# harmony-one/harmony

Hardware: AMD Instinct MI355X
Metric: BLS12-381 aggregate-verifies/sec (committee=4096) (higher is better)
Workload: dtype u64; 1 GPU; config2: committee=4096 masked aggregate + pairing verify, batch=262144/step, masks Bernoulli(0.9) seed 42, 48B staking commit payloads; parallelism=dp1 (per-shard replicas, no collective)

## Files before the change

### harmony_amd/core.py

```python
import ctypes
import os

_DIR = os.path.dirname(os.path.abspath(__file__))
_SO = os.environ.get("HBLS_SO", os.path.join(_DIR, "libhbls.so"))

HBLS_OK = 1
HBLS_FALSE = 0
HBLS_ERR = -1
HBLS_ERR_NOGPU = -2
HBLS_ERR_BADINPUT = -3
HBLS_NOQUORUM = -4
NOQUORUM = HBLS_NOQUORUM
TWO_THIRDS_DEC = 666666666666666667


class HblsError(RuntimeError):
    pass


class NoGpuError(HblsError):
    pass


class BadInputError(HblsError, ValueError):
# ... 35 lines not shown
                                       ctypes.c_size_t, ctypes.c_char_p]
    lib.hbls_msm_g1_committee.argtypes = [ctypes.c_void_p, ctypes.c_char_p,
                                          ctypes.c_char_p]
    lib.hbls_batch_agg_verify_partials.argtypes = [
        ctypes.c_void_p, ctypes.c_char_p, ctypes.c_char_p, ctypes.c_size_t,
        ctypes.c_char_p, ctypes.c_char_p, ctypes.c_size_t, ctypes.c_size_t,
        ctypes.POINTER(ctypes.c_int32)]
    lib.hbls_stream_create.restype = ctypes.c_void_p
    lib.hbls_stream_create.argtypes = [ctypes.c_void_p, ctypes.c_int]
    lib.hbls_stream_free.argtypes = [ctypes.c_void_p]
    lib.hbls_stream_set_rounds.argtypes = [
        ctypes.c_void_p, ctypes.POINTER(ctypes.c_uint32), ctypes.c_int,
        ctypes.c_char_p, ctypes.c_size_t]
    lib.hbls_stream_process.argtypes = [
        ctypes.c_void_p, ctypes.POINTER(ctypes.c_uint32),
        ctypes.POINTER(ctypes.c_uint32), ctypes.c_char_p,
        ctypes.POINTER(ctypes.c_uint32), ctypes.c_int,
        ctypes.c_size_t, ctypes.POINTER(ctypes.c_int32)]
    lib.hbls_stream_check.argtypes = [
        ctypes.c_void_p, ctypes.POINTER(ctypes.c_uint32), ctypes.c_int,
        ctypes.POINTER(ctypes.c_int32)]
    lib.hbls_stream_check_submit.argtypes = [
        ctypes.c_void_p, ctypes.POINTER(ctypes.c_uint32), ctypes.c_int]
    lib.hbls_stream_check_poll.argtypes = [
        ctypes.c_void_p, ctypes.POINTER(ctypes.c_int32)]
    lib.hbls_stream_get.argtypes = [ctypes.c_void_p, ctypes.c_uint32,
                                    ctypes.c_char_p, ctypes.c_char_p]
    lib.hbls_stream_set_verify_mode.argtypes = [ctypes.c_void_p, ctypes.c_int]
    lib.hbls_batch_verify_votes_grouped.argtypes = [
        ctypes.c_void_p, ctypes.POINTER(ctypes.c_uint32),
        ctypes.POINTER(ctypes.c_uint32), ctypes.c_char_p, ctypes.c_char_p,
        ctypes.c_size_t, ctypes.c_size_t, ctypes.c_size_t,
        ctypes.POINTER(ctypes.c_int32)]
    lib.hbls_vote_key_sums.argtypes = [
        ctypes.c_void_p, ctypes.POINTER(ctypes.c_uint32),
        ctypes.POINTER(ctypes.c_uint32), ctypes.c_size_t, ctypes.c_char_p,
        ctypes.POINTER(ctypes.c_int32)]
    lib.hbls_batch_verify_votes_multi.argtypes = [
        ctypes.c_void_p, ctypes.POINTER(ctypes.c_uint32),
        ctypes.POINTER(ctypes.c_uint32), ctypes.c_char_p, ctypes.c_char_p,
        ctypes.c_size_t, ctypes.c_size_t, ctypes.POINTER(ctypes.c_int32)]
    lib.hbls_stream_process_multi.argtypes = [
        ctypes.c_void_p, ctypes.POINTER(ctypes.c_uint32),
        ctypes.POINTER(ctypes.c_uint32), ctypes.POINTER(ctypes.c_uint32),
        ctypes.c_char_p, ctypes.POINTER(ctypes.c_uint32), ctypes.c_int,
        ctypes.c_size_t, ctypes.POINTER(ctypes.c_int32)]
    lib.hbls_rlc_last_stats.argtypes = [ctypes.POINTER(ctypes.c_uint32)]
    lib.hbls_rlc_last_stats.restype = None
    lib.hbls_set_agg_verify_mode.argtypes = [ctypes.c_int]
    lib.hbls_set_aggrlc_threshold.argtypes = [ctypes.c_int]
    lib.hbls_set_aggrlc_threshold.restype = None
    lib.hbls_aggrlc_last_stats.argtypes = [ctypes.POINTER(ctypes.c_uint32)]
    lib.hbls_aggrlc_last_stats.restype = None
    u64p, u32p, i32p = (ctypes.POINTER(t) for t in
                        (ctypes.c_uint64, ctypes.c_uint32, ctypes.c_int32))
    lib.hbls_committee_set_quorum.argtypes = [ctypes.c_void_p, u64p, ctypes.c_uint64]
    lib.hbls_mask_power.argtypes = [ctypes.c_void_p, ctypes.c_char_p, ctypes.c_size_t,
                                    u64p, u32p]
    lib.hbls_agg_verify_quorum.argtypes = lib.hbls_agg_verify.argtypes
    lib.hbls_batch_agg_verify_quorum.argtypes = lib.hbls_batch_agg_verify.argtypes
    lib.hbls_batch_seal_verify_quorum.argtypes = lib.hbls_batch_seal_verify.argtypes
    lib.hbls_stream_power.argtypes = [ctypes.c_void_p, u32p, ctypes.c_int,
                                      u64p, u32p, i32p]
    lib.hbls_last_stage_ns.argtypes = [ctypes.c_int]
    lib.hbls_copy_bench_ns.restype = ctypes.c_uint64
    lib.hbls_copy_bench_ns.argtypes = [ctypes.c_size_t]
    lib.hbls_fpmul_bench_waves.restype = ctypes.c_double
    lib.hbls_fpmul_bench_waves.argtypes = [ctypes.c_int, ctypes.c_int]
    return lib


_lib = _load()


def _check(rc, what):
    if rc == HBLS_ERR_NOGPU:
        raise NoGpuError(f"{what}: no AMD GPU available (product path requires gfx950)")
    if rc == HBLS_ERR_BADINPUT:
        raise BadInputError(f"{what}: bad input")
    if rc < 0:
        raise HblsError(f"{what}: error {rc}")
    return rc


def version() -> str:
    return _lib.hbls_version().decode()


def device_count() -> int:
    return _lib.hbls_device_count()


def init(device=-1):
    _check(_lib.hbls_init(device), "hbls_init")


def last_kernel_ns() -> int:
    return _lib.hbls_last_kernel_ns()


def last_stage_ns(i: int) -> int:
    return _lib.hbls_last_stage_ns(i)


def set_g2_cofactor_mode(fast: bool):
    _lib.hbls_set_g2_cofactor_mode(int(fast))


def set_coop_threshold(n: int):
    _lib.hbls_set_coop_threshold(n)


def rlc_chunk_size() -> int:
    return _lib.hbls_rlc_chunk_size()


def rlc_last_stats():
    out = (ctypes.c_uint32 * 4)()
    _lib.hbls_rlc_last_stats(out)
    return list(out)


def set_agg_verify_mode(mode: int):
    _check(_lib.hbls_set_agg_verify_mode(mode), "set_agg_verify_mode")


def set_aggrlc_threshold(n: int):
    _lib.hbls_set_aggrlc_threshold(n)


def aggrlc_chunk_size() -> int:
    return _lib.hbls_aggrlc_chunk_size()


def aggrlc_last_stats():
    out = (ctypes.c_uint32 * 3)()
    _lib.hbls_aggrlc_last_stats(out)
    return list(out)


def pk_from_sk(sk32: bytes) -> bytes:
    out = ctypes.create_string_buffer(48)
    _check(_lib.hbls_pk_from_sk(sk32, out), "pk_from_sk")
    return out.raw


def batch_pk_from_sk(sks: bytes, batch: int) -> bytes:
    out = ctypes.create_string_buffer(48 * batch)
    _check(_lib.hbls_batch_pk_from_sk(sks, batch, out), "batch_pk_from_sk")
    return out.raw


def sign_hash(sk32: bytes, msg: bytes) -> bytes:
    out = ctypes.create_string_buffer(96)
    _check(_lib.hbls_sign_hash(sk32, msg, len(msg), out), "sign_hash")
    return out.raw


def batch_sign(sks: bytes, msgs: bytes, mlen: int, batch: int) -> bytes:
    out = ctypes.create_string_buffer(96 * batch)
    _check(_lib.hbls_batch_sign(sks, msgs, mlen, batch, out), "batch_sign")
    return out.raw


def hash_to_g2(msg: bytes) -> bytes:
    out = ctypes.create_string_buffer(96)
    _check(_lib.hbls_hash_to_g2(msg, len(msg), out), "hash_to_g2")
    return out.raw


def batch_hash_to_g2(msgs: bytes, mlen: int, batch: int) -> bytes:
    out = ctypes.create_string_buffer(96 * batch)
    _check(_lib.hbls_batch_hash_to_g2(msgs, mlen, batch, out), "batch_hash_to_g2")
    return out.raw


def verify_hash(pk48: bytes, sig96: bytes, msg: bytes) -> bool:
    rc = _lib.hbls_verify_hash(pk48, sig96, msg, len(msg))
    return _check(rc, "verify_hash") == HBLS_OK


def g1_add(a: bytes, b: bytes) -> bytes:
    out = ctypes.create_string_buffer(48)
    _check(_lib.hbls_g1_add(a, b, out), "g1_add")
    return out.raw


def g1_sub(a: bytes, b: bytes) -> bytes:
    out = ctypes.create_string_buffer(48)
    _check(_lib.hbls_g1_sub(a, b, out), "g1_sub")
    return out.raw


# ... 334 lines not shown
```

### harmony_amd/csrc/hbls_aggrlc.inc

```

#define AGGRLC_CHUNK 64
#define AGGRLC_WINDOWS 8

__global__ void k_aggrlc_pow2(g1aff_t *p2) {
    int k = blockIdx.x * blockDim.x + threadIdx.x;
    if (k >= 64) return;
    g1_t base, p;
    fp_load(base.x, BLS_G1_X); fp_load(base.y, BLS_G1_Y); fp_one(base.z);
    g1_neg(p, base);
    for (int j = 0; j < k; j++) g1_dbl(p, p);
    g1aff_t a;
    g1_to_affine(a, p);
    p2[k] = a;
}

__global__ void k_aggrlc_miller(const g1_t *aggpubs, const g2_t *hms, const g2aff_t *sigs,
                                const int32_t *sig_flags, const int32_t *hm_ok,
                                const uint64_t *scalars, const g1aff_t *gtab,
                                fp12_t *F, int32_t *elig, int32_t *results, int batch) {
    int i = blockIdx.x * blockDim.x + threadIdx.x;
    if (i >= batch) return;
    fp12_t f;
    fp12_one(f);
    elig[i] = 0;
// ... 30 lines not shown
      fp_mul(zi, ti, A.z);
      fp_sqr(zi2, zi);
      fp_mul(zi3, zi2, zi);
      fp_mul(ca.x, C.x, zi2);
      fp_mul(ca.y, C.y, zi3); }
    g2aff_t ha;
    g2_t hmc = hms[i];
    g2_to_affine(ha, hmc);
    miller_loop2(f, ha, pa, sigs[i], ca);
    F[i] = f;
    elig[i] = 1;
    results[i] = 1;
}

__global__ void __launch_bounds__(AGGRLC_CHUNK) k_aggrlc_chunk_prod(
        const fp12_t *F, const int32_t *elig, int batch, int nchunks,
        fp12_t *FC, int32_t *ccnt, int32_t *cforce) {
    int c = blockIdx.x;
    if (c >= nchunks) return;
    __shared__ fp12_t red[AGGRLC_CHUNK];
    size_t i = (size_t)c * AGGRLC_CHUNK + threadIdx.x;
    int e = i < (size_t)batch ? elig[i] : 0;
    if (e == 1) red[threadIdx.x] = F[i];
    else fp12_one(red[threadIdx.x]);
    int cnt = __syncthreads_count(e != 0);
    int force = __syncthreads_or(e == 2);
    for (int s = AGGRLC_CHUNK / 2; s > 0; s >>= 1) {
        if (threadIdx.x < s) {
            fp12_t t;
            fp12_mul(t, red[threadIdx.x], red[threadIdx.x + s]);
            red[threadIdx.x] = t;
        }
        __syncthreads();
    }
    if (threadIdx.x == 0) {
        FC[c] = red[0];
        ccnt[c] = cnt;
        cforce[c] = force ? 1 : 0;
    }
}

__global__ void k_aggrlc_final(const fp12_t *FC, const int32_t *ccnt,
                               const int32_t *cforce, int32_t *verdict, int nchunks) {
    int c = blockIdx.x * blockDim.x + threadIdx.x;
    if (c >= nchunks) return;
    if (cforce[c]) { verdict[c] = 0; return; }
    if (ccnt[c] == 0) { verdict[c] = 1; return; }
    fp12_t f = FC[c];
    fp12_conj(f, f);
    final_exp(f, f);
    verdict[c] = fp12_is_one(f) ? 1 : 0;
}

__global__ void k_verify_sel(const uint32_t *sel, int nsel, const g1_t *aggpubs,
                             const g2_t *hms, const g2aff_t *sigs,
                             const int32_t *sig_flags, const int32_t *hm_ok,
                             int32_t *results, int batch) {
    int j = blockIdx.x * blockDim.x + threadIdx.x;
    if (j >= nsel) return;
    uint32_t i = sel[j];
    if (i >= (uint32_t)batch) return;
    if (!hm_ok[i] || sig_flags[i] == 0) { results[i] = HBLS_ERR_BADINPUT; return; }
    g2aff_t dummy;
    bool sig_inf = sig_flags[i] == 2;
    results[i] = verify_pairing(aggpubs[i], hms[i], sig_inf ? dummy : sigs[i], sig_inf);
}


static thread_local uint32_t g_aggrlc_stats[3] = {0, 0, 0};
extern "C" void hbls_aggrlc_last_stats(uint32_t out[3]) {
    for (int i = 0; i < 3; i++) out[i] = g_aggrlc_stats[i];
}
static void aggrlc_stats_reset(void) {
    for (int i = 0; i < 3; i++) g_aggrlc_stats[i] = 0;
}
extern "C" int hbls_aggrlc_chunk_size(void) { return AGGRLC_CHUNK; }

static int g_agg_verify_mode = -2;
#define AGGRLC_DEFAULT_THRESHOLD 131072
static int g_aggrlc_threshold = AGGRLC_DEFAULT_THRESHOLD;
static int agg_verify_mode(void) {
    if (g_agg_verify_mode == -2) {
        const char *e = getenv("HBLS_AGG_VERIFY_MODE");
        int m = e ? atoi(e) : -1;
        g_agg_verify_mode = (m == 0 || m == 1) ? m : -1;
    }
    return g_agg_verify_mode;
}
extern "C" int hbls_set_agg_verify_mode(int mode) {
    if (mode < -1 || mode > 1) return HBLS_ERR_BADINPUT;
    g_agg_verify_mode = mode;
    return HBLS_OK;
}
extern "C" void hbls_set_aggrlc_threshold(int n) {
    g_aggrlc_threshold = n < 0 ? AGGRLC_DEFAULT_THRESHOLD : n;
}

static g1aff_t *g_aggrlc_gtab = nullptr;
static int aggrlc_init_tables(void) {
    if (g_aggrlc_gtab) return HBLS_OK;
    const size_t m = AGGRLC_WINDOWS * 255;
    DevBuf dp2(64 * sizeof(g1aff_t)), dwj(m * sizeof(g1_t)), dwi(m);
    g1aff_t *d_gt = nullptr;
    if (dp2.err || dwj.err || dwi.err) return HBLS_ERR;
    HIP_OK(hipMalloc(&d_gt, m * sizeof(g1aff_t)));
    hipLaunchKernelGGL(k_aggrlc_pow2, dim3(1), dim3(64), 0, 0, dp2.as<g1aff_t>());
    hipLaunchKernelGGL(k_wtab_build_jac, dim3(1), dim3(64), 0, 0,
                       dp2.as<g1aff_t>(), 64, dwj.as<g1_t>(), AGGRLC_WINDOWS);
    hipLaunchKernelGGL(k_wtab_to_affine, dim3((int)((m + 255) / 256)), dim3(256), 0, 0,
                       dwj.as<g1_t>(), d_gt, dwi.as<uint8_t>(), m);
    std::vector<uint8_t> winf(m);
    bool ok = hipDeviceSynchronize() == hipSuccess &&
              hipMemcpy(winf.data(), dwi.p, m, hipMemcpyDeviceToHost) == hipSuccess;
    for (size_t k = 0; ok && k < m; k++)
        if (winf[k]) ok = false;
    if (!ok) { hipFree(d_gt); return HBLS_ERR; }
    g_aggrlc_gtab = d_gt;
    return HBLS_OK;
}

static bool aggrlc_wanted(size_t batch) {
    int m = agg_verify_mode();
    if (m == 0 || !g_aggrlc_gtab) return false;
    if (batch > RLC_MAX_ITEMS || (long long)batch < (long long)g_aggrlc_threshold) return false;
    if (m == 1) return true;
    return (int)batch > coop_threshold() && rf_mode() == 0 && !use_batch_affine();
}

static int aggrlc_verify(const g1_t *d_agg, const g2_t *d_hm, const g2aff_t *d_saff,
                         const int32_t *d_sflags, const int32_t *d_hok,
                         int32_t *d_res, size_t batch) {
    size_t nc = (batch + AGGRLC_CHUNK - 1) / AGGRLC_CHUNK;
    std::vector<uint64_t> scalars(batch);
    if (!rlc_draw_scalars(scalars.data(), batch)) return AGGRLC_FALLBACK;
    DevBuf dsc(batch * 8), dF(batch * sizeof(fp12_t)), delig(batch * 4);
    DevBuf dFC(nc * sizeof(fp12_t)), dcs(3 * nc * 4);
    if (dsc.err || dF.err || delig.err || dFC.err || dcs.err) {
        (void)hipGetLastError();
        return AGGRLC_FALLBACK;
    }
    HIP_OK(hipMemcpy(dsc.p, scalars.data(), batch * 8, hipMemcpyHostToDevice));
    int32_t *d_ccnt = dcs.as<int32_t>(), *d_cforce = d_ccnt + nc, *d_verdict = d_cforce + nc;
    hipEvent_t ev[4];
    for (int i = 0; i < 4; i++) (void)hipEventCreate(&ev[i]);
    (void)hipEventRecord(ev[0], 0);
    hipLaunchKernelGGL(k_aggrlc_miller, dim3((uint32_t)((batch + 63) / 64)), dim3(64), 0, 0,
                       d_agg, d_hm, d_saff, d_sflags, d_hok, dsc.as<uint64_t>(),
                       g_aggrlc_gtab, dF.as<fp12_t>(), delig.as<int32_t>(), d_res, (int)batch);
    (void)hipEventRecord(ev[1], 0);
    hipLaunchKernelGGL(k_aggrlc_chunk_prod, dim3((uint32_t)nc), dim3(AGGRLC_CHUNK), 0, 0,
                       dF.as<fp12_t>(), delig.as<int32_t>(), (int)batch, (int)nc,
                       dFC.as<fp12_t>(), d_ccnt, d_cforce);
    (void)hipEventRecord(ev[2], 0);
    hipLaunchKernelGGL(k_aggrlc_final, dim3((uint32_t)((nc + 63) / 64)), dim3(64), 0, 0,
                       dFC.as<fp12_t>(), d_ccnt, d_cforce, d_verdict, (int)nc);
    (void)hipEventRecord(ev[3], 0);
    std::vector<int32_t> hc(3 * nc);
    hipError_t e = hipMemcpy(hc.data(), dcs.p, 3 * nc * 4, hipMemcpyDeviceToHost);
    if (e == hipSuccess) e = hipGetLastError();
    for (int i = 0; i < 3; i++) {
        float ms = 0;
        if (e == hipSuccess) (void)hipEventElapsedTime(&ms, ev[i], ev[i + 1]);
        g_stage_ns[4 + i] = (uint64_t)(ms * 1e6);
    }
    for (int i = 0; i < 4; i++) (void)hipEventDestroy(ev[i]);
    HIP_OK(e);

    std::vector<uint32_t> failed;
    for (size_t c = 0; c < nc; c++) {
        if (hc[c] <= 0) continue;
        g_aggrlc_stats[0]++;
        if (hc[2 * nc + c] == 1) continue;
        g_aggrlc_stats[1]++;
        failed.push_back((uint32_t)c);
    }
    if (failed.empty()) return HBLS_OK;

    std::vector<int32_t> helig(batch);
    HIP_OK(hipMemcpy(helig.data(), delig.p, batch * 4, hipMemcpyDeviceToHost));
    std::vector<uint32_t> sel;
    for (uint32_t c : failed)
        for (size_t i = (size_t)c * AGGRLC_CHUNK;
             i < batch && i < ((size_t)c + 1) * AGGRLC_CHUNK; i++)
            if (helig[i]) sel.push_back((uint32_t)i);
    size_t ns = sel.size();
    g_aggrlc_stats[2] = (uint32_t)ns;
    if (!ns) return HBLS_OK;
    DevBuf dsel(ns * 4);
    if (dsel.err) return HBLS_ERR;
    HIP_OK(hipMemcpy(dsel.p, sel.data(), ns * 4, hipMemcpyHostToDevice));
    hipLaunchKernelGGL(k_verify_sel, dim3((uint32_t)((ns + 63) / 64)), dim3(64), 0, 0,
                       dsel.as<uint32_t>(), (int)ns, d_agg, d_hm, d_saff, d_sflags, d_hok,
                       d_res, (int)batch);
    HIP_OK(hipGetLastError());
    return HBLS_OK;
}
```

### harmony_amd/csrc/hbls_dev.hip

```cpp
#include <hip/hip_runtime.h>
#include <stdint.h>
#include <string.h>
#include <stdio.h>
#include <stdlib.h>
#include "../../oracle/bls_consts.h"
#include "../../include/hbls.h"

typedef unsigned __int128 u128;

#define DEV __device__ __forceinline__
#define DEVN __device__ __noinline__

struct fp_t { uint64_t l[6]; };
struct fp2_t { fp_t a, b; };

DEV bool fp_is_zero(const fp_t &x) {
    return (x.l[0] | x.l[1] | x.l[2] | x.l[3] | x.l[4] | x.l[5]) == 0;
}
DEV bool fp_eq(const fp_t &x, const fp_t &y) {
    uint64_t d = 0;
#pragma unroll
    for (int i = 0; i < 6; i++) d |= x.l[i] ^ y.l[i];
    return d == 0;
}
// ... 2105 lines not shown
static int aggrlc_init_tables(void);
static bool aggrlc_wanted(size_t batch);
static void aggrlc_stats_reset(void);

#define HIP_OK(expr) do { hipError_t _e = (expr); if (_e != hipSuccess) { \
    fprintf(stderr, "hbls: %s failed: %s\n", #expr, hipGetErrorString(_e)); return HBLS_ERR; } } while (0)
#define HIP_OKP(expr) do { hipError_t _e = (expr); if (_e != hipSuccess) { \
    fprintf(stderr, "hbls: %s failed: %s\n", #expr, hipGetErrorString(_e)); return nullptr; } } while (0)

extern "C" int hbls_device_count(void) {
    int n = 0;
    if (hipGetDeviceCount(&n) != hipSuccess) return 0;
    return n;
}

extern "C" int hbls_init(int device) {
    int n = hbls_device_count();
    if (n <= 0) return HBLS_ERR_NOGPU;
    if (device >= 0) {
        if (device >= n) return HBLS_ERR_BADINPUT;
        if (hipSetDevice(device) != hipSuccess) return HBLS_ERR;
        g_device = device;
    } else {
        hipGetDevice(&g_device);
    }
    void *p = nullptr;
    if (hipMalloc(&p, 64) != hipSuccess) return HBLS_ERR;
    hipFree(p);
    g_init_rc = HBLS_OK;
    (void)aggrlc_init_tables();
    return HBLS_OK;
}

extern "C" void hbls_set_g2_cofactor_mode(int fast) { g_fast_cofactor = fast; }
extern "C" const char *hbls_version(void) { return "hbls 0.1 (gfx950)"; }
extern "C" uint64_t hbls_last_kernel_ns(void) { return g_last_ns; }
extern "C" uint64_t hbls_last_stage_ns(int i) { return (i >= 0 && i < 8) ? g_stage_ns[i] : 0; }

static int require_gpu(void) {
    if (g_init_rc != HBLS_OK) {
        if (hbls_init(-1) != HBLS_OK) return HBLS_ERR_NOGPU;
    }
    return HBLS_OK;
}

struct DevBuf {
    void *p = nullptr;
    hipError_t err = hipSuccess;
    explicit DevBuf(size_t n) { err = hipMalloc(&p, n ? n : 1); }
    ~DevBuf() { if (p) hipFree(p); }
    template <typename T> T *as() const { return (T *)p; }
};

struct Timer {
    hipEvent_t a, b;
    Timer() { hipEventCreate(&a); hipEventCreate(&b); hipEventRecord(a, 0); }
    void stop_and_store() {
        hipEventRecord(b, 0);
        hipEventSynchronize(b);
        float ms = 0;
        hipEventElapsedTime(&ms, a, b);
        g_last_ns = (uint64_t)(ms * 1e6);
        hipEventDestroy(a); hipEventDestroy(b);
    }
};

extern "C" int hbls_batch_pk_from_sk(const uint8_t *sks32, size_t batch, uint8_t *pks48) {
    int rc = require_gpu();
    if (rc != HBLS_OK) return rc;
    DevBuf dsk(batch * 32), dpk(batch * 48), dok(batch * 4);
    if (dsk.err || dpk.err || dok.err) return HBLS_ERR;
    HIP_OK(hipMemcpy(dsk.p, sks32, batch * 32, hipMemcpyHostToDevice));
    Timer tm;
    int nb = (int)((batch + 63) / 64);
    hipLaunchKernelGGL(k_pk_from_sk, dim3(nb), dim3(64), 0, 0,
                       dsk.as<uint8_t>(), dpk.as<uint8_t>(), dok.as<int32_t>(), (int)batch);
    tm.stop_and_store();
    HIP_OK(hipGetLastError());
    HIP_OK(hipMemcpy(pks48, dpk.p, batch * 48, hipMemcpyDeviceToHost));
    std::vector<int32_t> ok(batch);
    HIP_OK(hipMemcpy(ok.data(), dok.p, batch * 4, hipMemcpyDeviceToHost));
    for (size_t i = 0; i < batch; i++)
        if (!ok[i]) return HBLS_ERR_BADINPUT;
    return HBLS_OK;
}

extern "C" int hbls_pk_from_sk(const uint8_t sk32[32], uint8_t pk48[48]) {
    return hbls_batch_pk_from_sk(sk32, 1, pk48);
}

extern "C" int hbls_batch_hash_to_g2(const uint8_t *msgs, size_t msg_len, size_t batch,
                                     uint8_t *out96s) {
    int rc = require_gpu();
    if (rc != HBLS_OK) return rc;
    DevBuf dm(batch * msg_len), dout(batch * sizeof(g2_t)), dok(batch * 4), dser(batch * 96);
    if (dm.err || dout.err || dok.err || dser.err) return HBLS_ERR;
    HIP_OK(hipMemcpy(dm.p, msgs, batch * msg_len, hipMemcpyHostToDevice));
    Timer tm;
    int nb = (int)((batch + 63) / 64);
    hipLaunchKernelGGL(k_hash_to_g2, dim3(nb), dim3(64), 0, 0,
                       dm.as<uint8_t>(), (int)msg_len, dout.as<g2_t>(), dok.as<int32_t>(),
                       (int)batch, g_fast_cofactor);
    hipLaunchKernelGGL(k_g2_serialize, dim3(nb), dim3(64), 0, 0,
                       dout.as<g2_t>(), dser.as<uint8_t>(), dok.as<int32_t>(), (int)batch);
    tm.stop_and_store();
    HIP_OK(hipGetLastError());
// ... 178 lines not shown
        DevBuf ones(bm);
        if (!ones.err) {
            std::vector<uint8_t> host_ones(bm, 0);
            for (size_t i = 0; i < n; i++) host_ones[i >> 3] |= 1 << (i & 7);
            if (hipMemcpy(ones.p, host_ones.data(), bm, hipMemcpyHostToDevice) == hipSuccess) {
                launch_mask_aggregate(c->d_table, (int)n, ones.as<uint8_t>(),
                                      (int)bm, (const g1_t *)nullptr, d_fs, 1,
                                      c->d_wtab, c->d_winf);
                if (hipDeviceSynchronize() == hipSuccess)
                    c->d_full_sum = d_fs;
            }
        }
        if (c->d_full_sum == nullptr) hipFree(d_fs);
    }
    return c;
}
extern "C" void hbls_committee_free(hbls_committee_t *c) {
    if (c) {
        hipFree(c->d_table);
        if (c->d_full_sum) hipFree(c->d_full_sum);
        if (c->d_wtab) hipFree(c->d_wtab);
        if (c->d_winf) hipFree(c->d_winf);
        if (c->d_power) hipFree(c->d_power);
        delete c;
    }
}
extern "C" size_t hbls_committee_size(const hbls_committee_t *c) { return c->n; }

extern "C" int hbls_mask_aggregate_g1(const hbls_committee_t *c, const uint8_t *bitmap,
                                      uint8_t out48[48]) {
    int rc = require_gpu();
    if (rc != HBLS_OK) return rc;
    size_t bm = (c->n + 7) / 8;
    DevBuf dbm(bm), dout(sizeof(g1_t)), dser(48);
    if (dbm.err || dout.err || dser.err) return HBLS_ERR;
    HIP_OK(hipMemcpy(dbm.p, bitmap, bm, hipMemcpyHostToDevice));
    Timer tm;
    launch_mask_aggregate(c->d_table, (int)c->n, dbm.as<uint8_t>(), (int)bm,
                          c->d_full_sum, dout.as<g1_t>(), 1,
                          c->d_wtab, c->d_winf);
    hipLaunchKernelGGL(k_g1_serialize, dim3(1), dim3(1), 0, 0,
                       dout.as<g1_t>(), dser.as<uint8_t>(), 1);
    tm.stop_and_store();
    HIP_OK(hipGetLastError());
    HIP_OK(hipMemcpy(out48, dser.p, 48, hipMemcpyDeviceToHost));
    return HBLS_OK;
}

static int aggrlc_verify(const g1_t *d_agg, const g2_t *d_hm, const g2aff_t *d_saff,
                         const int32_t *d_sflags, const int32_t *d_hok,
                         int32_t *d_res, size_t batch);
#define AGGRLC_FALLBACK 2

static int run_agg_verify_pipeline(const hbls_committee_t *c, const uint8_t *d_bm,
                                   const uint8_t *d_sig, const uint8_t *d_msg,
                                   size_t msg_len, size_t batch, int32_t *results) {
    size_t bm = (c->n + 7) / 8;
    DevBuf dagg(batch * sizeof(g1_t)), dhm(batch * sizeof(g2_t));
    DevBuf dsaff(batch * sizeof(g2aff_t)), dsflags(batch * 4), dhok(batch * 4), dres(batch * 4);
    if (dagg.err || dhm.err || dsaff.err || dsflags.err || dhok.err || dres.err)
        return HBLS_ERR;
    int nb = (int)((batch + 63) / 64);
    aggrlc_stats_reset();
    hipEvent_t ev[5];
    for (int i = 0; i < 5; i++) (void)hipEventCreate(&ev[i]);
    (void)hipEventRecord(ev[0], 0);
    launch_mask_aggregate(c->d_table, (int)c->n, d_bm, (int)bm,
                                         c->d_full_sum, dagg.as<g1_t>(), (int)batch,
                                         c->d_wtab, c->d_winf);
    (void)hipEventRecord(ev[1], 0);
    if ((int)batch <= coop_threshold()) {
        int nbc = (int)((batch + CV_ITEMS - 1) / CV_ITEMS);
        LAUNCH_COOP(k_hash_to_g2_coop, batch, d_msg, (int)msg_len, dhm.as<g2_t>(), dhok.as<int32_t>(),
                           (int)batch, g_fast_cofactor);
    } else {
        hipLaunchKernelGGL(k_hash_to_g2, dim3(nb), dim3(64), 0, 0,
                           d_msg, (int)msg_len, dhm.as<g2_t>(), dhok.as<int32_t>(),
                           (int)batch, g_fast_cofactor);
    }
    (void)hipEventRecord(ev[2], 0);
    if ((int)batch <= coop_threshold()) {
        int nbc = (int)((batch + CV_ITEMS - 1) / CV_ITEMS);
        LAUNCH_COOP(k_g2_decompress_coop, batch, d_sig, dsaff.as<g2aff_t>(), dsflags.as<int32_t>(), (int)batch);
    } else {
        hipLaunchKernelGGL(k_g2_decompress, dim3(nb), dim3(64), 0, 0,
                           d_sig, dsaff.as<g2aff_t>(), dsflags.as<int32_t>(), (int)batch);
    }
    (void)hipEventRecord(ev[3], 0);
    int arc = AGGRLC_FALLBACK;
    if (aggrlc_wanted(batch)) {
        arc = aggrlc_verify(dagg.as<g1_t>(), dhm.as<g2_t>(), dsaff.as<g2aff_t>(),
                            dsflags.as<int32_t>(), dhok.as<int32_t>(), dres.as<int32_t>(), batch);
        if (arc != HBLS_OK && arc != AGGRLC_FALLBACK) return arc;
    }
    if (arc == HBLS_OK) {
    } else if ((int)batch <= coop_threshold()) {
        int nbc = (int)((batch + CV_ITEMS - 1) / CV_ITEMS);
        LAUNCH_COOP(k_verify_coop, batch, dagg.as<g1_t>(), dhm.as<g2_t>(), dsaff.as<g2aff_t>(),
                           dsflags.as<int32_t>(), dhok.as<int32_t>(), dres.as<int32_t>(), (int)batch);
    } else if (rf_mode() == 0 && use_batch_affine()) {
        DevBuf dpa(batch * sizeof(g1aff_t)), dpi(batch * 4), dha(batch * sizeof(g2aff_t));
        if (dpa.err || dpi.err || dha.err) return HBLS_ERR;
        int nba = (int)((batch + 64 * BA_K - 1) / (64 * BA_K));
        hipLaunchKernelGGL(k_g1_batch_affine, dim3(nba), dim3(64), 0, 0,
                           dagg.as<g1_t>(), dpa.as<g1aff_t>(), dpi.as<int32_t>(), (int)batch);
        hipLaunchKernelGGL(k_g2_batch_affine, dim3(nba), dim3(64), 0, 0,
                           dhm.as<g2_t>(), dha.as<g2aff_t>(), dhok.as<int32_t>(), (int)batch);
        hipLaunchKernelGGL(k_verify_aff, dim3(nb), dim3(64), 0, 0,
                           dpa.as<g1aff_t>(), dpi.as<int32_t>(), dha.as<g2aff_t>(),
                           dsaff.as<g2aff_t>(), dsflags.as<int32_t>(), dhok.as<int32_t>(),
                           dres.as<int32_t>(), (int)batch);
        HIP_OK(hipDeviceSynchronize());
    } else {
        LAUNCH_VERIFY_SCALAR(nb, dagg.as<g1_t>(), dhm.as<g2_t>(), dsaff.as<g2aff_t>(),
                           dsflags.as<int32_t>(), dhok.as<int32_t>(), dres.as<int32_t>(), (int)batch);
    }
    (void)hipEventRecord(ev[4], 0);
    HIP_OK(hipEventSynchronize(ev[4]));
    float ms_total = 0, ms = 0;
    (void)hipEventElapsedTime(&ms_total, ev[0], ev[4]);
    g_last_ns = (uint64_t)(ms_total * 1e6);
    for (int i = 0; i < 4; i++) {
        (void)hipEventElapsedTime(&ms, ev[i], ev[i + 1]);
        g_stage_ns[i] = (uint64_t)(ms * 1e6);
    }
    for (int i = 0; i < 5; i++) (void)hipEventDestroy(ev[i]);
    HIP_OK(hipGetLastError());
    HIP_OK(hipMemcpy(results, dres.p, batch * 4, hipMemcpyDeviceToHost));
    return HBLS_OK;
}

extern "C" int hbls_batch_agg_verify(const hbls_committee_t *c, const uint8_t *bitmaps,
                                     const uint8_t *sigs96, const uint8_t *msgs,
                                     size_t msg_len, size_t batch, int32_t *results) {
    int rc = require_gpu();
    if (rc != HBLS_OK) return rc;
    size_t bm = (c->n + 7) / 8;
    DevBuf dbm(batch * bm), dsig(batch * 96), dmsg(batch * msg_len);
    if (dbm.err || dsig.err || dmsg.err) return HBLS_ERR;
    HIP_OK(hipMemcpy(dbm.p, bitmaps, batch * bm, hipMemcpyHostToDevice));
    HIP_OK(hipMemcpy(dsig.p, sigs96, batch * 96, hipMemcpyHostToDevice));
    HIP_OK(hipMemcpy(dmsg.p, msgs, batch * msg_len, hipMemcpyHostToDevice));
    return run_agg_verify_pipeline(c, dbm.as<uint8_t>(), dsig.as<uint8_t>(),
                                   dmsg.as<uint8_t>(), msg_len, batch, results);
}

extern "C" int hbls_agg_verify(const hbls_committee_t *c, const uint8_t *bitmap,
                               const uint8_t sig96[96], const uint8_t *msg, size_t msg_len) {
    int32_t r;
    int rc = hbls_batch_agg_verify(c, bitmap, sig96, msg, msg_len, 1, &r);
    if (rc != HBLS_OK) return rc;
    return r;
}

extern "C" int hbls_batch_verify_votes(const hbls_committee_t *c, const uint32_t *key_idx,
                                       const uint8_t *sigs96, const uint8_t *msgs,
                                       size_t msg_len, size_t batch, int32_t *results) {
    int rc = require_gpu();
    if (rc != HBLS_OK) return rc;
    DevBuf didx(batch * 4), dsig(batch * 96), dmsg(batch * msg_len);
    DevBuf dhm(batch * sizeof(g2_t)), dsaff(batch * sizeof(g2aff_t));
    DevBuf dsflags(batch * 4), dhok(batch * 4), dres(batch * 4);
    size_t gsz = rf_mode() ? batch : 1;
    DevBuf gpub(gsz * sizeof(g1_t)), ghm(gsz * sizeof(g2_t)), gok(gsz * 4);
    if (didx.err || dsig.err || dmsg.err || dhm.err || dsaff.err || dsflags.err ||
        dhok.err || dres.err || gpub.err || ghm.err || gok.err) return HBLS_ERR;
    HIP_OK(hipMemcpy(didx.p, key_idx, batch * 4, hipMemcpyHostToDevice));
    HIP_OK(hipMemcpy(dsig.p, sigs96, batch * 96, hipMemcpyHostToDevice));
    HIP_OK(hipMemcpy(dmsg.p, msgs, batch * msg_len, hipMemcpyHostToDevice));
    Timer tm;
    int nb = (int)((batch + 63) / 64);
    if ((int)batch <= coop_threshold()) {
        int nbc = (int)((batch + CV_ITEMS - 1) / CV_ITEMS);
        LAUNCH_COOP(k_hash_to_g2_coop, batch, dmsg.as<uint8_t>(), (int)msg_len, dhm.as<g2_t>(), dhok.as<int32_t>(),
                           (int)batch, g_fast_cofactor);
    } else {
        hipLaunchKernelGGL(k_hash_to_g2, dim3(nb), dim3(64), 0, 0,
                           dmsg.as<uint8_t>(), (int)msg_len, dhm.as<g2_t>(), dhok.as<int32_t>(),
                           (int)batch, g_fast_cofactor);
    }
    if ((int)batch <= coop_threshold()) {
        int nbc = (int)((batch + CV_ITEMS - 1) / CV_ITEMS);
        LAUNCH_COOP(k_g2_decompress_coop, batch, dsig.as<uint8_t>(), dsaff.as<g2aff_t>(), dsflags.as<int32_t>(), (int)batch);
    } else {
        hipLaunchKernelGGL(k_g2_decompress, dim3(nb), dim3(64), 0, 0,
                           dsig.as<uint8_t>(), dsaff.as<g2aff_t>(), dsflags.as<int32_t>(), (int)batch);
    }
    if ((int)batch <= coop_threshold()) {
        int nbc = (int)((batch + CV_ITEMS - 1) / CV_ITEMS);
        LAUNCH_COOP(k_verify_votes_coop, batch, c->d_table, (int)c->n, didx.as<uint32_t>(), dhm.as<g2_t>(),
                           (const uint32_t *)nullptr,
                           dsaff.as<g2aff_t>(), dsflags.as<int32_t>(), dhok.as<int32_t>(),
                           dres.as<int32_t>(), (int)batch);
    } else {
#ifdef HBLS_RF
        if (rf_mode() >= 1 && rf_mode() <= 3) {
            LAUNCH_VOTES_SCALAR_RF(nb, c->d_table, (int)c->n, didx.as<uint32_t>(),
// ... 1479 lines not shown
```

### include/hbls.h

```cpp
#ifndef HBLS_H
#define HBLS_H

#include <stddef.h>
#include <stdint.h>

#ifdef __cplusplus
extern "C" {
#endif

enum {
    HBLS_OK = 1,
    HBLS_FALSE = 0,
    HBLS_ERR = -1,
    HBLS_ERR_NOGPU = -2,
    HBLS_ERR_BADINPUT = -3,
    HBLS_NOQUORUM = -4,
};

#define HBLS_TWO_THIRDS_DEC 666666666666666667ULL

int hbls_init(int device);

int hbls_device_count(void);

// ... 83 lines not shown
int hbls_mask_power(const hbls_committee_t *c, const uint8_t *bitmaps, size_t batch,
                    uint64_t *power_out, uint32_t *count_out);

int hbls_batch_agg_verify_quorum(const hbls_committee_t *c, const uint8_t *bitmaps,
                                 const uint8_t *sigs96, const uint8_t *msgs,
                                 size_t msg_len, size_t batch, int32_t *results);
int hbls_batch_seal_verify_quorum(const hbls_committee_t *c,
                                  const uint8_t *sig_bitmaps, size_t blob_len,
                                  const uint8_t *msgs, size_t msg_len,
                                  size_t batch, int32_t *results);
int hbls_agg_verify_quorum(const hbls_committee_t *c, const uint8_t *bitmap,
                           const uint8_t sig96[96], const uint8_t *msg, size_t msg_len);

int hbls_g2_aggregate(const uint8_t *sigs96, size_t n, uint8_t out96[96]);

typedef struct hbls_stream hbls_stream_t;
hbls_stream_t *hbls_stream_create(const hbls_committee_t *c, int max_rounds);
void hbls_stream_free(hbls_stream_t *s);
int hbls_stream_set_rounds(hbls_stream_t *s, const uint32_t *slots, int k,
                           const uint8_t *payloads, size_t payload_len);
int hbls_stream_process(hbls_stream_t *s, const uint32_t *key_idx,
                        const uint32_t *round_idx, const uint8_t *sigs96,
                        const uint32_t *active_slots, int n_active,
                        size_t batch, int32_t *results);
int hbls_stream_set_verify_mode(hbls_stream_t *s, int mode);
int hbls_stream_check(hbls_stream_t *s, const uint32_t *slots, int k, int32_t *ok);
int hbls_stream_check_submit(hbls_stream_t *s, const uint32_t *slots, int k);
int hbls_stream_check_poll(hbls_stream_t *s, int32_t *ok);
int hbls_stream_get(hbls_stream_t *s, uint32_t slot, uint8_t *bitmap_out,
                    uint8_t agg96_out[96]);

int hbls_stream_power(hbls_stream_t *s, const uint32_t *slots, int k,
                      uint64_t *power_out, uint32_t *count_out, int32_t *quorum_out);


int hbls_vote_key_sums(const hbls_committee_t *c, const uint32_t *key_off,
                       const uint32_t *key_idx, size_t batch,
                       uint8_t *out48s, int32_t *ok);

int hbls_batch_verify_votes_multi(const hbls_committee_t *c, const uint32_t *key_off,
                                  const uint32_t *key_idx, const uint8_t *sigs96,
                                  const uint8_t *msgs, size_t msg_len, size_t batch,
                                  int32_t *results);

int hbls_stream_process_multi(hbls_stream_t *s, const uint32_t *key_off,
                              const uint32_t *key_idx, const uint32_t *round_idx,
                              const uint8_t *sigs96, const uint32_t *active_slots,
                              int n_active, size_t batch, int32_t *results);

int hbls_set_agg_verify_mode(int mode);
void hbls_set_aggrlc_threshold(int min_batch);
int hbls_aggrlc_chunk_size(void);
void hbls_aggrlc_last_stats(uint32_t out[3]);

int hbls_batch_keccak256(const uint8_t *msgs, size_t msg_len, size_t batch,
                         uint8_t *out32s);

const char *hbls_version(void);
double hbls_mad_peak_ops(void);
uint64_t hbls_last_kernel_ns(void);

#ifdef __cplusplus
}
#endif
#endif
```

Measured before the change: 680,300 aggregate-verifies/sec.

## Overlap input uploads with kernels, cooperative final exp, lower RLC threshold

Adds a cooperative multi-lane final-exponentiation kernel for the aggregated-RLC path and makes it the default. Host-to-device uploads of messages, signatures and bitmaps now go through a separate non-blocking stream, each fenced with an event just before the kernel that consumes it, and mask aggregation is moved after hash-to-G2 and decompress so later uploads can overlap earlier kernels. Also lowers the default batch threshold for the aggregated RLC path and adds host-side timing instrumentation plus a selftest. The per-chunk final exp was a small serial tail, and the risks are extra stream/event overhead and more complexity.

```diff
diff --git a/harmony_amd/core.py b/harmony_amd/core.py
--- a/harmony_amd/core.py
+++ b/harmony_amd/core.py
@@ -111,6 +111,10 @@
     lib.hbls_set_aggrlc_threshold.restype = None
     lib.hbls_aggrlc_last_stats.argtypes = [ctypes.POINTER(ctypes.c_uint32)]
     lib.hbls_aggrlc_last_stats.restype = None
+    lib.hbls_set_aggrlc_final.argtypes = [ctypes.c_int]
+    lib.hbls_aggrlc_final_selftest.argtypes = [ctypes.c_int]
+    lib.hbls_last_host_ns.restype = ctypes.c_uint64
+    lib.hbls_last_host_ns.argtypes = [ctypes.c_int]
     u64p, u32p, i32p = (ctypes.POINTER(t) for t in
                         (ctypes.c_uint64, ctypes.c_uint32, ctypes.c_int32))
     lib.hbls_committee_set_quorum.argtypes = [ctypes.c_void_p, u64p, ctypes.c_uint64]
@@ -198,6 +202,18 @@
     return list(out)
 
 
+def set_aggrlc_final(kernel: int):
+    _check(_lib.hbls_set_aggrlc_final(kernel), "set_aggrlc_final")
+
+
+def aggrlc_final_selftest(nchunks: int) -> int:
+    return _check(_lib.hbls_aggrlc_final_selftest(nchunks), "aggrlc_final_selftest")
+
+
+def last_host_ns(i: int) -> int:
+    return _lib.hbls_last_host_ns(i)
+
+
 def pk_from_sk(sk32: bytes) -> bytes:
     out = ctypes.create_string_buffer(48)
     _check(_lib.hbls_pk_from_sk(sk32, out), "pk_from_sk")
diff --git a/harmony_amd/csrc/hbls_aggrlc.inc b/harmony_amd/csrc/hbls_aggrlc.inc
--- a/harmony_amd/csrc/hbls_aggrlc.inc
+++ b/harmony_amd/csrc/hbls_aggrlc.inc
@@ -106,6 +106,41 @@
     verdict[c] = fp12_is_one(f) ? 1 : 0;
 }
 
+template <int ITEMS>
+__global__ void __launch_bounds__(ITEMS * CV_LANES) k_aggrlc_final_coop(
+        const fp12_t *FC, const int32_t *ccnt, const int32_t *cforce,
+        int32_t *verdict, int nchunks) {
+    __shared__ uint64_t arena[ITEMS][CV_STRIDE64];
+    __shared__ int32_t pre[ITEMS];
+    const int sub = threadIdx.x / CV_LANES;
+    const int q = threadIdx.x % CV_LANES;
+    const int c = blockIdx.x * ITEMS + sub;
+    lds_fp2 *A = (lds_fp2 *)arena[sub];
+    if (q == 0) {
+        int32_t r = -2;
+        if (c >= nchunks) r = -1;
+        else if (cforce[c]) r = 0;
+        else if (ccnt[c] == 0) r = 1;
+        pre[sub] = r;
+        fp12_t f;
+        if (r == -2) f = FC[c];
+        else fp12_one(f);
+        cv_st_fp12(A, CV_F0, f);
+    }
+    __syncthreads();
+    cv_fp12_conj(A, q, CV_F0, CV_F0);
+    cv_final_exp(A, q);
+    if (q == 0) {
+        int32_t r = pre[sub];
+        if (r == -2) {
+            fp12_t f;
+            cv_ld_fp12(A, CV_F0, f);
+            r = fp12_is_one(f) ? 1 : 0;
+        }
+        if (r != -1) verdict[c] = r;
+    }
+}
+
 __global__ void k_verify_sel(const uint32_t *sel, int nsel, const g1_t *aggpubs,
                              const g2_t *hms, const g2aff_t *sigs,
                              const int32_t *sig_flags, const int32_t *hm_ok,
@@ -131,7 +166,7 @@
 extern "C" int hbls_aggrlc_chunk_size(void) { return AGGRLC_CHUNK; }
 
 static int g_agg_verify_mode = -2;
-#define AGGRLC_DEFAULT_THRESHOLD 131072
+#define AGGRLC_DEFAULT_THRESHOLD 16384
 static int g_aggrlc_threshold = AGGRLC_DEFAULT_THRESHOLD;
 static int agg_verify_mode(void) {
     if (g_agg_verify_mode == -2) {
@@ -148,6 +183,98 @@
 }
 extern "C" void hbls_set_aggrlc_threshold(int n) {
     g_aggrlc_threshold = n < 0 ? AGGRLC_DEFAULT_THRESHOLD : n;
+}
+
+#define AGGRLC_FINAL_DEFAULT 16
+static int g_aggrlc_final = -2;
+static int aggrlc_final_kernel(void) {
+    if (g_aggrlc_final == -2) {
+        const char *e = getenv("HBLS_AGGRLC_FINAL");
+        int k = e ? atoi(e) : AGGRLC_FINAL_DEFAULT;
+        g_aggrlc_final = (k == 0 || k == 8 || k == 16) ? k : AGGRLC_FINAL_DEFAULT;
+    }
+    return g_aggrlc_final;
+}
+extern "C" int hbls_set_aggrlc_final(int kernel) {
+    if (kernel == -1) kernel = AGGRLC_FINAL_DEFAULT;
+    if (kernel != 0 && kernel != 8 && kernel != 16) return HBLS_ERR_BADINPUT;
+    g_aggrlc_final = kernel;
+    return HBLS_OK;
+}
+static void launch_aggrlc_final(int kernel, const fp12_t *d_FC, const int32_t *d_ccnt,
+                                const int32_t *d_cforce, int32_t *d_verdict, int nc) {
+    if (kernel == 16)
+        hipLaunchKernelGGL(k_aggrlc_final_coop<16>, dim3((uint32_t)((nc + 15) / 16)),
+                           dim3(16 * CV_LANES), 0, 0, d_FC, d_ccnt, d_cforce, d_verdict, nc);
+    else if (kernel == 8)
+        hipLaunchKernelGGL(k_aggrlc_final_coop<8>, dim3((uint32_t)((nc + 7) / 8)),
+                           dim3(8 * CV_LANES), 0, 0, d_FC, d_ccnt, d_cforce, d_verdict, nc);
+    else
+        hipLaunchKernelGGL(k_aggrlc_final, dim3((uint32_t)((nc + 63) / 64)), dim3(64), 0, 0,
+                           d_FC, d_ccnt, d_cforce, d_verdict, nc);
+}
+
+__global__ void k_aggrlc_final_fill(fp12_t *FC, int32_t *ccnt, int32_t *cforce, int nchunks) {
+    int c = blockIdx.x * blockDim.x + threadIdx.x;
+    if (c >= nchunks) return;
+    int kind = c % 8;
+    fp_t one;
+    fp_one(one);
+    fp_t co[12];
+    for (int k = 0; k < 12; k++) {
+        fp_t t;
+        fp_zero(t);
+        uint32_t m = (uint32_t)c * 12u + (uint32_t)k + 3u;
+        for (int b = 31; b >= 0; b--) {
+            fp_dbl(t, t);
+            if ((m >> b) & 1u) fp_add(t, t, one);
+        }
+        fp_sqr(t, t);
+        fp_add(t, t, one);
+        fp_sqr(t, t);
+        co[k] = t;
+    }
+    fp12_t f;
+    fp2_t *s = &f.c0.c0;
+    for (int k = 0; k < 6; k++) { s[k].a = co[2 * k]; s[k].b = co[2 * k + 1]; }
+    if (kind == 1 || kind == 5)
+        for (int k = 3; k < 6; k++) { fp_zero(s[k].a); fp_zero(s[k].b); }
+    if (kind == 2) fp12_one(f);
+    FC[c] = f;
+    ccnt[c] = kind == 3 ? 0 : 1 + c % 64;
+    cforce[c] = (kind == 4 || kind == 5) ? 1 : 0;
+}
+
+extern "C" int hbls_aggrlc_final_selftest(int nchunks) {
+    int rc = require_gpu();
+    if (rc != HBLS_OK) return rc;
+    if (nchunks < 1 || nchunks > (1 << 20)) return HBLS_ERR_BADINPUT;
+    size_t nc = (size_t)nchunks;
+    DevBuf dFC(nc * sizeof(fp12_t)), dcs(2 * nc * 4), dv(3 * nc * 4);
+    if (dFC.err || dcs.err || dv.err) return HBLS_ERR;
+    int32_t *d_ccnt = dcs.as<int32_t>(), *d_cforce = d_ccnt + nc;
+    HIP_OK(hipMemset(dv.p, 0xff, 3 * nc * 4));
+    hipLaunchKernelGGL(k_aggrlc_final_fill, dim3((uint32_t)((nc + 63) / 64)), dim3(64), 0, 0,
+                       dFC.as<fp12_t>(), d_ccnt, d_cforce, nchunks);
+    const int kernels[3] = { 0, 16, 8 };
+    for (int k = 0; k < 3; k++)
+        launch_aggrlc_final(kernels[k], dFC.as<fp12_t>(), d_ccnt, d_cforce,
+                            dv.as<int32_t>() + k * nc, nchunks);
+    HIP_OK(hipGetLastError());
+    std::vector<int32_t> v(3 * nc);
+    HIP_OK(hipMemcpy(v.data(), dv.p, 3 * nc * 4, hipMemcpyDeviceToHost));
+    int zeros = 0, ones = 0;
+    for (size_t c = 0; c < nc; c++) {
+        int kind = (int)(c % 8);
+        int want = (kind == 1 || kind == 2 || kind == 3) ? 1 : 0;
+        if (v[c] != want) return HBLS_ERR;
+        if (v[c]) ones++; else zeros++;
+    }
+    if (nc >= 2 && (!zeros || !ones)) return HBLS_ERR;
+    int diff = 0;
+    for (size_t c = 0; c < nc; c++)
+        if (v[nc + c] != v[c] || v[2 * nc + c] != v[c]) diff++;
+    return diff;
 }
 
 static g1aff_t *g_aggrlc_gtab = nullptr;
@@ -187,13 +314,19 @@
     size_t nc = (batch + AGGRLC_CHUNK - 1) / AGGRLC_CHUNK;
     std::vector<uint64_t> scalars(batch);
     if (!rlc_draw_scalars(scalars.data(), batch)) return AGGRLC_FALLBACK;
+    FreeClock fclk;
+    uint64_t t_alloc = host_now_ns();
     DevBuf dsc(batch * 8), dF(batch * sizeof(fp12_t)), delig(batch * 4);
     DevBuf dFC(nc * sizeof(fp12_t)), dcs(3 * nc * 4);
+    g_host_ns[0] += host_now_ns() - t_alloc;
+    FreeClockArm farm(fclk);
     if (dsc.err || dF.err || delig.err || dFC.err || dcs.err) {
         (void)hipGetLastError();
         return AGGRLC_FALLBACK;
     }
-    HIP_OK(hipMemcpy(dsc.p, scalars.data(), batch * 8, hipMemcpyHostToDevice));
+    EventSet<1> up;
+    if (up.err != hipSuccess) return HBLS_ERR;
+    HIP_OK(upload_then_wait(dsc.p, scalars.data(), batch * 8, up[0]));
     int32_t *d_ccnt = dcs.as<int32_t>(), *d_cforce = d_ccnt + nc, *d_verdict = d_cforce + nc;
     hipEvent_t ev[4];
     for (int i = 0; i < 4; i++) (void)hipEventCreate(&ev[i]);
@@ -206,8 +339,8 @@
                        dF.as<fp12_t>(), delig.as<int32_t>(), (int)batch, (int)nc,
                        dFC.as<fp12_t>(), d_ccnt, d_cforce);
     (void)hipEventRecord(ev[2], 0);
-    hipLaunchKernelGGL(k_aggrlc_final, dim3((uint32_t)((nc + 63) / 64)), dim3(64), 0, 0,
-                       dFC.as<fp12_t>(), d_ccnt, d_cforce, d_verdict, (int)nc);
+    launch_aggrlc_final(aggrlc_final_kernel(), dFC.as<fp12_t>(), d_ccnt, d_cforce,
+                        d_verdict, (int)nc);
     (void)hipEventRecord(ev[3], 0);
     std::vector<int32_t> hc(3 * nc);
     hipError_t e = hipMemcpy(hc.data(), dcs.p, 3 * nc * 4, hipMemcpyDeviceToHost);
diff --git a/harmony_amd/csrc/hbls_dev.hip b/harmony_amd/csrc/hbls_dev.hip
--- a/harmony_amd/csrc/hbls_dev.hip
+++ b/harmony_amd/csrc/hbls_dev.hip
@@ -2181,6 +2181,77 @@
     template <typename T> T *as() const { return (T *)p; }
 };
 
+#include <chrono>
+static thread_local uint64_t g_host_ns[5] = {0};
+static thread_local bool g_host_open = false;
+static inline uint64_t host_now_ns(void) {
+    return (uint64_t)std::chrono::duration_cast<std::chrono::nanoseconds>(
+        std::chrono::steady_clock::now().time_since_epoch()).count();
+}
+extern "C" uint64_t hbls_last_host_ns(int i) { return (i >= 0 && i < 5) ? g_host_ns[i] : 0; }
+struct HostSpan {
+    int i; uint64_t t0;
+    explicit HostSpan(int idx) : i(idx), t0(host_now_ns()) {}
+    ~HostSpan() { g_host_ns[i] += host_now_ns() - t0; }
+};
+struct HostCall {
+    bool owner; uint64_t t0;
+    HostCall() : owner(!g_host_open), t0(0) {
+        if (!owner) return;
+        g_host_open = true;
+        for (int i = 0; i < 5; i++) g_host_ns[i] = 0;
+        t0 = host_now_ns();
+    }
+    ~HostCall() {
+        if (!owner) return;
+        g_host_ns[4] = host_now_ns() - t0;
+        g_host_open = false;
+    }
+};
+struct FreeClock {
+    uint64_t t0 = 0; bool armed = false;
+    ~FreeClock() { if (armed) g_host_ns[3] += host_now_ns() - t0; }
+};
+struct FreeClockArm {
+    FreeClock &fc;
+    explicit FreeClockArm(FreeClock &f) : fc(f) {}
+    ~FreeClockArm() { fc.t0 = host_now_ns(); fc.armed = true; }
+};
+
+static hipStream_t g_upload_stream = nullptr;
+static std::once_flag g_upload_flag;
+static hipStream_t upload_stream(void) {
+    std::call_once(g_upload_flag, [] {
+        hipStream_t s = nullptr;
+        if (hipStreamCreateWithFlags(&s, hipStreamNonBlocking) == hipSuccess)
+            g_upload_stream = s;
+        else
+            (void)hipGetLastError();
+    });
+    return g_upload_stream;
+}
+static hipError_t upload_then_wait(void *dst, const void *src, size_t n, hipEvent_t done) {
+    HostSpan sp(1);
+    hipStream_t s = upload_stream();
+    hipError_t e = hipMemcpyAsync(dst, src, n, hipMemcpyHostToDevice, s);
+    if (e == hipSuccess) e = hipEventRecord(done, s);
+    if (e == hipSuccess) e = hipStreamWaitEvent(0, done, 0);
+    return e;
+}
+template <int N> struct EventSet {
+    hipEvent_t e[N];
+    hipError_t err = hipSuccess;
+    EventSet() {
+        for (int i = 0; i < N; i++) {
+            e[i] = nullptr;
+            hipError_t r = hipEventCreate(&e[i]);
+            if (r != hipSuccess) err = r;
+        }
+    }
+    ~EventSet() { for (int i = 0; i < N; i++) if (e[i]) (void)hipEventDestroy(e[i]); }
+    hipEvent_t operator[](int i) const { return e[i]; }
+};
+
 struct Timer {
     hipEvent_t a, b;
     Timer() { hipEventCreate(&a); hipEventCreate(&b); hipEventRecord(a, 0); }
@@ -2465,23 +2536,32 @@
                          int32_t *d_res, size_t batch);
 #define AGGRLC_FALLBACK 2
 
+struct AggHostSrc { const uint8_t *bitmaps, *sigs, *msgs; };
+
 static int run_agg_verify_pipeline(const hbls_committee_t *c, const uint8_t *d_bm,
                                    const uint8_t *d_sig, const uint8_t *d_msg,
-                                   size_t msg_len, size_t batch, int32_t *results) {
+                                   size_t msg_len, size_t batch, int32_t *results,
+                                   const AggHostSrc *src = nullptr) {
+    HostCall hcall;
     size_t bm = (c->n + 7) / 8;
+    FreeClock fclk;
+    uint64_t t_alloc = host_now_ns();
     DevBuf dagg(batch * sizeof(g1_t)), dhm(batch * sizeof(g2_t));
     DevBuf dsaff(batch * sizeof(g2aff_t)), dsflags(batch * 4), dhok(batch * 4), dres(batch * 4);
+    g_host_ns[0] += host_now_ns() - t_alloc;
+    FreeClockArm farm(fclk);
     if (dagg.err || dhm.err || dsaff.err || dsflags.err || dhok.err || dres.err)
         return HBLS_ERR;
     int nb = (int)((batch + 63) / 64);
     aggrlc_stats_reset();
-    hipEvent_t ev[5];
-    for (int i = 0; i < 5; i++) (void)hipEventCreate(&ev[i]);
-    (void)hipEventRecord(ev[0], 0);
-    launch_mask_aggregate(c->d_table, (int)c->n, d_bm, (int)bm,
-                                         c->d_full_sum, dagg.as<g1_t>(), (int)batch,
-                                         c->d_wtab, c->d_winf);
-    (void)hipEventRecord(ev[1], 0);
+    for (int i = 4; i < 7; i++) g_stage_ns[i] = 0;
+    EventSet<8> ev;
+    EventSet<3> up;
+    if (ev.err != hipSuccess || up.err != hipSuccess) return HBLS_ERR;
+    uint64_t t_launch = host_now_ns();
+
+    if (src) HIP_OK(upload_then_wait((void *)d_msg, src->msgs, batch * msg_len, up[0]));
+    (void)hipEventRecord(ev[2], 0);
     if ((int)batch <= coop_threshold()) {
         int nbc = (int)((batch + CV_ITEMS - 1) / CV_ITEMS);
         LAUNCH_COOP(k_hash_to_g2_coop, batch, d_msg, (int)msg_len, dhm.as<g2_t>(), dhok.as<int32_t>(),
@@ -2491,7 +2571,10 @@
                            d_msg, (int)msg_len, dhm.as<g2_t>(), dhok.as<int32_t>(),
                            (int)batch, g_fast_cofactor);
     }
-    (void)hipEventRecord(ev[2], 0);
+    (void)hipEventRecord(ev[3], 0);
+
+    if (src) HIP_OK(upload_then_wait((void *)d_sig, src->sigs, batch * 96, up[1]));
+    (void)hipEventRecord(ev[4], 0);
     if ((int)batch <= coop_threshold()) {
         int nbc = (int)((batch + CV_ITEMS - 1) / CV_ITEMS);
         LAUNCH_COOP(k_g2_decompress_coop, batch, d_sig, dsaff.as<g2aff_t>(), dsflags.as<int32_t>(), (int)batch);
@@ -2499,7 +2582,16 @@
         hipLaunchKernelGGL(k_g2_decompress, dim3(nb), dim3(64), 0, 0,
                            d_sig, dsaff.as<g2aff_t>(), dsflags.as<int32_t>(), (int)batch);
     }
-    (void)hipEventRecord(ev[3], 0);
+    (void)hipEventRecord(ev[5], 0);
+
+    if (src) HIP_OK(upload_then_wait((void *)d_bm, src->bitmaps, batch * bm, up[2]));
+    (void)hipEventRecord(ev[0], 0);
+    launch_mask_aggregate(c->d_table, (int)c->n, d_bm, (int)bm,
+                                         c->d_full_sum, dagg.as<g1_t>(), (int)batch,
+                                         c->d_wtab, c->d_winf);
+    (void)hipEventRecord(ev[1], 0);
+
+    (void)hipEventRecord(ev[6], 0);
     int arc = AGGRLC_FALLBACK;
     if (aggrlc_wanted(batch)) {
         arc = aggrlc_verify(dagg.as<g1_t>(), dhm.as<g2_t>(), dsaff.as<g2aff_t>(),
@@ -2528,18 +2620,18 @@
         LAUNCH_VERIFY_SCALAR(nb, dagg.as<g1_t>(), dhm.as<g2_t>(), dsaff.as<g2aff_t>(),
                            dsflags.as<int32_t>(), dhok.as<int32_t>(), dres.as<int32_t>(), (int)batch);
     }
-    (void)hipEventRecord(ev[4], 0);
-    HIP_OK(hipEventSynchronize(ev[4]));
+    (void)hipEventRecord(ev[7], 0);
+    HIP_OK(hipEventSynchronize(ev[7]));
     float ms_total = 0, ms = 0;
-    (void)hipEventElapsedTime(&ms_total, ev[0], ev[4]);
+    (void)hipEventElapsedTime(&ms_total, ev[2], ev[7]);
     g_last_ns = (uint64_t)(ms_total * 1e6);
     for (int i = 0; i < 4; i++) {
-        (void)hipEventElapsedTime(&ms, ev[i], ev[i + 1]);
+        (void)hipEventElapsedTime(&ms, ev[2 * i], ev[2 * i + 1]);
         g_stage_ns[i] = (uint64_t)(ms * 1e6);
     }
-    for (int i = 0; i < 5; i++) (void)hipEventDestroy(ev[i]);
     HIP_OK(hipGetLastError());
     HIP_OK(hipMemcpy(results, dres.p, batch * 4, hipMemcpyDeviceToHost));
+    g_host_ns[2] += host_now_ns() - t_launch;
     return HBLS_OK;
 }
 
@@ -2548,14 +2640,17 @@
                                      size_t msg_len, size_t batch, int32_t *results) {
     int rc = require_gpu();
     if (rc != HBLS_OK) return rc;
+    HostCall hcall;
     size_t bm = (c->n + 7) / 8;
+    FreeClock fclk;
+    uint64_t t_alloc = host_now_ns();
     DevBuf dbm(batch * bm), dsig(batch * 96), dmsg(batch * msg_len);
+    g_host_ns[0] += host_now_ns() - t_alloc;
+    FreeClockArm farm(fclk);
     if (dbm.err || dsig.err || dmsg.err) return HBLS_ERR;
-    HIP_OK(hipMemcpy(dbm.p, bitmaps, batch * bm, hipMemcpyHostToDevice));
-    HIP_OK(hipMemcpy(dsig.p, sigs96, batch * 96, hipMemcpyHostToDevice));
-    HIP_OK(hipMemcpy(dmsg.p, msgs, batch * msg_len, hipMemcpyHostToDevice));
+    AggHostSrc src = { bitmaps, sigs96, msgs };
     return run_agg_verify_pipeline(c, dbm.as<uint8_t>(), dsig.as<uint8_t>(),
-                                   dmsg.as<uint8_t>(), msg_len, batch, results);
+                                   dmsg.as<uint8_t>(), msg_len, batch, results, &src);
 }
 
 extern "C" int hbls_agg_verify(const hbls_committee_t *c, const uint8_t *bitmap,
diff --git a/include/hbls.h b/include/hbls.h
--- a/include/hbls.h
+++ b/include/hbls.h
@@ -159,6 +159,8 @@
 void hbls_set_aggrlc_threshold(int min_batch);
 int hbls_aggrlc_chunk_size(void);
 void hbls_aggrlc_last_stats(uint32_t out[3]);
+int hbls_set_aggrlc_final(int kernel);
+int hbls_aggrlc_final_selftest(int nchunks);
 
 int hbls_batch_keccak256(const uint8_t *msgs, size_t msg_len, size_t batch,
                          uint8_t *out32s);
@@ -166,6 +168,7 @@
 const char *hbls_version(void);
 double hbls_mad_peak_ops(void);
 uint64_t hbls_last_kernel_ns(void);
+uint64_t hbls_last_host_ns(int i);
 
 #ifdef __cplusplus
 }
```

Result: faster. 738,500 aggregate-verifies/sec (median of 6 runs) (+8.6%).
